# fernandezdaniel/MOBOCMF

Hardware: AMD Instinct MI355X
Metric: ELBO steps/sec (MFDGP d=8 M=512 N=8192 S=8) (higher is better)
Workload: dtype f64

## Files before the change

### mobocmf_amd/csrc/api.hip

```cpp
#include "common.h"

static const mobocmf_tuning kDefaultTuning = {(uint32_t)sizeof(mobocmf_tuning), 384, 512, 0, 0, 1024, 32, 0, 1, 0};
static thread_local const mobocmf_tuning* t_tuning = nullptr;
static thread_local void* const* t_probe = nullptr;
const mobocmf_tuning& tune() { return t_tuning ? *t_tuning : kDefaultTuning; }
bool tuning_ok(const mobocmf_tuning* t) {
    if (!t) return true;
    return t->struct_size == sizeof(mobocmf_tuning) && t->small_gemm_max >= 1 && t->small_gemm_max <= 512 &&
           t->small_panel_max >= 1 && t->small_panel_max <= 512 && (t->tile_rows == 0 || t->tile_rows == 64 || t->tile_rows == 128) &&
           t->pair_mode >= 0 && t->pair_mode <= 2 && t->mid_gemm_max >= 0 && t->mid_gemm_max <= 4096 &&
           (t->mid_gemm_waves == 4 || t->mid_gemm_waves == 8 || t->mid_gemm_waves == 32) &&
           (t->syrk_workgroups == 0 || (t->syrk_workgroups >= 16 && t->syrk_workgroups <= 4096)) &&
           (t->sparse_backward == 0 || t->sparse_backward == 1) && (t->potrf_cols == 0 || t->potrf_cols == 1 || t->potrf_cols == 4);
}
TuneScope::TuneScope(const mobocmf_tuning* t, void* const* probe) : prev_t(t_tuning), prev_p(t_probe) {
    t_tuning = t;
    t_probe = probe;
}
TuneScope::~TuneScope() {
    t_tuning = prev_t;
    t_probe = prev_p;
}
void probe_at(int i, hipStream_t s) {
    if (t_probe && i < MOBOCMF_PROBE_EVENTS && t_probe[i]) (void)hipEventRecord((hipEvent_t)t_probe[i], s);
// ... 344 lines not shown
    TRY(launch_moments_bwd_prep(g_mean, g_var, P.knn, P.q, P.varraw, desc->branch, desc->min_var, D.N, Np, B.gmu, B.gv,
                                B.gv2, B.cgv, nclamped, c.nclamped ? 1 : 0, (int32_t*)act, s));
    int da_parts = 0;
    {
        GemmArgs ga = gemm_args(c.U, Mp, P.C, Np, B.dA, Np, Mp, Np, Mp, TRI_LOWER_A, 2.0);
        ga.bscale = B.gv; ga.epi = EPI_DA; ga.avec = c.a; ga.gmu = B.gmu; ga.cgv = B.cgv; ga.Aaux = P.A;
        ga.Kreal = D.M;
        ga.rowdot_part = desc->params_const ? nullptr : B.dapart;
        ga.colact = act;
        ga.rm = panel_tile_rows(Mp, Np);
        set_pairing(ga);
        probe_at(3, s);
        TRY(launch_gemm(ga, false, 1, s));
        probe_at(4, s);
        da_parts = desc->params_const ? 0 : gemm_rowdot_parts(ga);
    }
    if (!desc->params_const) {
        probe_at(5, s);
        if (desc->branch == 0) TRY(weighted_syrk_pair(P.A, Np, B.gv, B.cgv, Mp, Np, B.slabs, B.slabs2, c.H, Hc, nclamped, act, s));
        else TRY(weighted_syrk(P.A, Np, B.gv, Mp, Np, B.slabs, c.H, nullptr, nullptr, act, s));
        probe_at(6, s);
    }
    {
        GemmArgs ga = gemm_args(c.LinvT, Mp, B.dA, Np, B.dK, Np, Mp, Np, Mp, TRI_UPPER_A, 1.0);
        ga.Kreal = D.M;
        ga.rm = panel_tile_rows(Mp, Np);
        set_pairing(ga);
        ga.colact = act;
        probe_at(7, s);
        TRY(launch_gemm(ga, false, 1, s));
        probe_at(8, s);
    }
    GramArgs g = {};
    g.kind = desc->kind; g.d = desc->d; g.zdiv = 1; g.Zx = Zx; g.zf = zf; g.M = D.M; g.hyp = hyp; g.Mp = Mp;
    g.xdiv = desc->xdiv; g.x = x; g.f = f; g.nbase = D.nbase;
    g.ldk = Np; g.Np = Np; g.G = B.dK; g.gknn = B.cgv; g.colact = act;
    g.hyp_part = B.hyp_part; g.df_part = B.df_part; g.dzf_part = B.dzf_part; g.dx_part = B.dx_part;
    TRY(launch_gram_bwd(g, desc->want_dx != 0, s));
    probe_at(10, s);
    SumTask tk[5];
    int nt = 0;
    if (da_parts > 0) tk[nt++] = {B.dapart, da_parts, Mp, nullptr, 0, 0, c.da, Mp, 0};
    tk[nt++] = {B.hyp_part, (int64_t)D.ggrid_mn.x * D.ggrid_mn.y, D.H, nullptr, 0, 0, g_hyp, D.H, 0};
    if (desc->kind == 1) {
        tk[nt++] = {B.df_part, D.ggrid_mn.y, Np, nullptr, 0, 0, g_f, D.N, 0};
        tk[nt++] = {B.dzf_part, D.ggrid_mn.x, Mp, nullptr, 0, 0, g_zf, D.M, 0};
    }
    if (desc->want_dx)
        tk[nt++] = {B.dx_part, D.ggrid_mn.y, D.nbase * desc->d, nullptr, 0, 0, g_x, D.nbase * desc->d, 0};
    return launch_sum_partials_multi(tk, nt, s);
}

int chain_backward(int n, const ChainWs& c, int64_t zs, const ChainIO& io, const Dims& D, const bool* zero, const int* acc,
                   const bool* fold, hipStream_t s) {
    const int Mp = D.Mp;
    const int64_t mm = (int64_t)Mp * Mp;
    double *G1 = c.W[0], *F = c.W[1], *Gm = c.W[2], *dU = c.W[3], *Wn = c.W[4], *T1 = c.W[5], *T4 = c.W[6], *T2 = c.W[7];
    bool any_clamp_branch = false;
    for (int z = 0; z < n; ++z) {
        if (zero[z]) {
            TRY(launch_zero32(c.H + z * zs, mm * 2, s));
            TRY(launch_zero32(c.Hc + z * zs, mm * 2, s));
            TRY(launch_zero32(c.da + z * zs, (int64_t)Mp * 2, s));
        }
        any_clamp_branch = any_clamp_branch || io.desc[z]->branch == 0;
    }
    for (int z = 0; z < n; ++z)
        if (io.desc[z]->branch != 0 && !zero[z] && (n > 1 || any_clamp_branch))
            TRY(launch_copy_block(c.H + z * zs, Mp, c.Hc + z * zs, Mp, Mp, Mp, s));
    const double* Hc = (n == 1 && io.desc[0]->branch != 0) ? c.H : c.Hc;
    {
        GemmArgs g1 = gemm_args(c.UT, Mp, c.H, Mp, G1, Mp, Mp, Mp, Mp, TRI_UPPER_A, 1.0);
        g1.Kreal = D.M;
        TRY(chain_gemm(g1, false, c, n, zs, s));
        TRY(launch_chain_glue_z(G1, Hc, c.U, c.da, c.a, io.g_kl, D.M, Mp, F, dU, c.da_tot, Wn, n, zs, s));
        GemmArgs gw = gemm_args(F, Mp, c.UT, Mp, Wn, Mp, Mp, Mp, Mp, TRI_UPPER_B, -1.0);
        gw.accumulate = 1;
        gw.Kreal = D.M;
        TRY(chain_gemm(gw, false, c, n, zs, s));
    }
    {
        GemmArgs ga = gemm_args(c.LinvT, Mp, dU, Mp, T1, Mp, Mp, Mp, Mp, TRI_UPPER_A | TRI_LOWER_B, 1.0);
        ga.lower_out = 1;
        ga.Kreal = D.M;
        GemmArgs gb = gemm_args(c.LinvT, Mp, Wn, Mp, T4, Mp, Mp, Mp, Mp, TRI_UPPER_A, 1.0);
        gb.Kreal = D.M;
        if (n > 1) {
            ga.zlayers = gb.zlayers = n;
            ga.zsA = ga.zsB = ga.zsC = gb.zsA = gb.zsB = gb.zsC = zs;
        }
        TRY(launch_gemm_auto_pair(ga, gb, c.slabs, c.slab_elems, s));
        TRY(launch_chain_outputs_z(T1, c.LSp, c.LinvT, c.da_tot, D.M, Mp, io.g_kl, io.g_LS, io.g_m, n, zs, s));
    }
    {
        GemmArgs gc = gemm_args(T4, Mp, c.Linv, Mp, T2, Mp, Mp, Mp, Mp, TRI_LOWER_B, 1.0);
        gc.Kreal = D.M;
        TRY(chain_gemm(gc, false, c, n, zs, s));
        TRY(launch_symmetrize_z(T2, Mp, Gm, n, zs, s));
    }
    SumTask tk[2 * MAX_ZL];
    int nt = 0;
    for (int z = 0; z < n; ++z) {
        const mobocmf_layer_desc* d = io.desc[z];
        GramArgs g = kmm_gram(d, D, io.Zx[z], io.zf[z], io.hyp[z]);
        g.G = Gm + z * zs; g.gknn = nullptr;
        g.hyp_part = c.hyp_part2 + z * zs; g.df_part = c.df_part2 + z * zs; g.dzf_part = c.dzf_part2 + z * zs;
        g.dx_part = nullptr;
        TRY(launch_gram_bwd(g, false, s));
        const int H = hyp_len(d->kind, d->d);
        tk[nt++] = {g.hyp_part, (int64_t)D.ggrid_mm.x * D.ggrid_mm.y, H, nullptr, 0, 0, io.g_hyp[z], H, acc[z]};
        if (d->kind == 1) {
            if (fold[z])
                tk[nt++] = {g.df_part, D.ggrid_mm.y, Mp, g.dzf_part, D.ggrid_mm.x, Mp, io.g_m[z - 1], D.M, 1,
                            acc[z] ? io.g_zf[z] : nullptr};
            else
                tk[nt++] = {g.df_part, D.ggrid_mm.y, Mp, g.dzf_part, D.ggrid_mm.x, Mp, io.g_zf[z], D.M, acc[z], nullptr};
        }
    }
    return launch_sum_partials_multi(tk, nt, s);
}

bool gram_rows_shape_ok(int32_t kind, int32_t d, int64_t n1, int64_t nbase2, int32_t xdiv) {
    return (kind == 0 || kind == 1) && d >= 1 && d <= MOBOCMF_MAX_D && n1 >= 1 && nbase2 >= 1 && xdiv >= 1 &&
           xdiv <= MOBOCMF_MAX_XDIV && n1 <= (int64_t)65535 * 64 && nbase2 <= 0x7fffffff;
}
int64_t gram_rows_part_elems(int32_t d, int64_t n1, int64_t nbase2, int32_t xdiv, int64_t* chunks_out = nullptr) {
    int64_t chunks;
    int groups, wb;
    gram_rows_geometry(n1, nbase2, xdiv, &chunks, &groups, &wb);
    if (chunks_out) *chunks_out = chunks;
    return chunks * n1 * d;
}
int gram_rows_partials(int kind, int d, const double* x1, const double* f1, int64_t n1, const double* x2, const double* f2,
                       int64_t nbase2, int xdiv, const double* hyp, const double* G, int64_t ldk, const int32_t* colact,
                       int symmetric, double* part, hipStream_t s) {
    GramRowsArgs g = {};
    g.kind = kind; g.d = d; g.xdiv = xdiv; g.symmetric = symmetric;
    g.x1 = x1; g.f1 = f1; g.n1 = n1; g.x2 = x2; g.f2 = f2; g.nbase2 = nbase2;
    g.hyp = hyp; g.G = G; g.ldk = ldk; g.colact = colact; g.part = part;
    return launch_gram_bwd_rows(g, s);
}
bool ranges_overlap(const void* a, size_t na, const void* b, size_t nb) {
    const uintptr_t pa = (uintptr_t)a, pb = (uintptr_t)b;
    return a && b && pa < pb + nb && pb < pa + na;
}
int panel_rows_partials(const mobocmf_layer_desc* desc, const Dims& D, const PanelBwd& B, const double* x, const double* f,
                        const double* Zx, const double* zf, const double* hyp, double* part, hipStream_t s) {
    return gram_rows_partials(desc->kind, desc->d, Zx, zf, D.M, x, f, D.nbase, desc->xdiv, hyp, B.dK, D.Np,
                              tune().sparse_backward ? B.blkact : nullptr, 0, part, s);
}
int chain_rows_partials(const mobocmf_layer_desc* desc, const Dims& D, const ChainWs& c, int z, int64_t zs, const double* Zx,
                        const double* zf, const double* hyp, double* part, hipStream_t s) {
    return gram_rows_partials(desc->kind, desc->d, Zx, zf, D.M, Zx, zf, D.M, 1, hyp, c.W[2] + z * zs, D.Mp, nullptr, 1, part, s);
}

bool same_chain_shape(int n, const mobocmf_layer_desc* const* d) {
    for (int z = 0; z < n; ++z)
        if (!valid_desc(d[z]) || d[z]->M != d[0]->M) return false;
    return true;
}

}

namespace {
int64_t gcd64(int64_t a, int64_t b) { while (b) { int64_t t = a % b; a = b; b = t; } return a; }
int64_t covpanel_cols(const mobocmf_layer_desc* d, int64_t Np) {
    const int64_t l = (int64_t)TILE / gcd64(TILE, d->xdiv) * d->xdiv;
    int64_t w = l * (2048 / l > 1 ? 2048 / l : 1);
    return w < Np ? w : Np;
}
struct CovWs { double *Knm, *AT, *CT, *Cv; };
// ... 45 lines not shown
    if (!valid_desc(desc) || desc->params_const || !x || !Zx || !hyp || !m || !L_S || !mean || !var || !kl || !info || !saved ||
        !scratch)
        return MOBOCMF_BAD_ARG;
    TuneScope tune_scope(desc->tuning, desc->probe_events);
    if (desc->kind == 1 && (!zf || !f)) return MOBOCMF_BAD_ARG;
    hipStream_t s = (hipStream_t)stream;
    Dims D = dims_of(desc);
    ChainWs c = {};
    PanelSaved P;
    PanelFwd F;
    if (!carve_single_saved(saved, saved_bytes, D, c, P) || !carve_single_fwd(scratch, scratch_bytes, D, c, F))
        return MOBOCMF_WORKSPACE_TOO_SMALL;
    ChainIO io = {};
    io.desc = &desc; io.Zx = &Zx; io.zf = &zf; io.hyp = &hyp; io.m = &m; io.L_S = &L_S; io.kl = &kl; io.info = &info;
    TRY(chain_forward(1, c, 0, io, D, s));
    return panel_forward(desc, D, c, P, F, x, f, Zx, zf, hyp, mean, var, s);
}

static int layer_backward_impl(const mobocmf_layer_desc* desc, const double* x, const double* f, const double* Zx,
                               const double* zf, const double* hyp, const double* m, const double* L_S,
                               const double* g_mean, const double* g_var, const double* g_kl, double* g_f, double* g_zf,
                               double* g_hyp, double* g_m, double* g_LS, double* g_x, void* saved, size_t saved_bytes,
                               void* scratch, size_t scratch_bytes, bool want_z, double* g_Zx, void* zws, size_t zws_bytes,
                               mobocmf_stream_t stream) {
    if ((want_z && (!g_Zx || !zws)) || !valid_desc(desc) || desc->params_const || !x || !Zx || !hyp || !g_mean || !g_var || !g_kl || !g_hyp || !g_m || !g_LS ||
        (desc->want_dx && !g_x) || !saved || !scratch)
        return MOBOCMF_BAD_ARG;
    TuneScope tune_scope(desc->tuning, desc->probe_events);
    if (desc->kind == 1 && (!zf || !g_zf || !f || !g_f)) return MOBOCMF_BAD_ARG;
    hipStream_t s = (hipStream_t)stream;
    Dims D = dims_of(desc);
    ChainWs c = {};
    PanelSaved P;
    PanelBwd B;
    if (!carve_single_saved(saved, saved_bytes, D, c, P) || !carve_single_bwd(scratch, scratch_bytes, D, desc, c, B))
        return MOBOCMF_WORKSPACE_TOO_SMALL;
    Bump bz(zws, zws_bytes);
    int64_t chp = 0, chc = 0;
    double *zp = nullptr, *zc = nullptr;
    if (want_z) {
        if (ranges_overlap(zws, zws_bytes, scratch, scratch_bytes) || ranges_overlap(zws, zws_bytes, saved, saved_bytes))
            return MOBOCMF_BAD_ARG;
        zp = bz.take(gram_rows_part_elems(desc->d, D.M, D.nbase, desc->xdiv, &chp));
        zc = bz.take(gram_rows_part_elems(desc->d, D.M, D.M, 1, &chc));
        if (!bz.ok) return MOBOCMF_WORKSPACE_TOO_SMALL;
    }
    TRY(panel_backward(desc, D, c, P, B, x, f, Zx, zf, hyp, g_mean, g_var, g_f, g_zf, g_hyp, g_x, s));
    if (want_z) TRY(panel_rows_partials(desc, D, B, x, f, Zx, zf, hyp, zp, s));
    ChainIO io = {};
    io.desc = &desc; io.Zx = &Zx; io.zf = &zf; io.hyp = &hyp; io.m = &m; io.L_S = &L_S;
    io.g_kl = &g_kl; io.g_zf = &g_zf; io.g_hyp = &g_hyp; io.g_m = &g_m; io.g_LS = &g_LS;
    const bool zero = false, fold = false;
    const int acc = 1;
    TRY(chain_backward(1, c, 0, io, D, &zero, &acc, &fold, s));
    if (!want_z) return MOBOCMF_OK;
    TRY(chain_rows_partials(desc, D, c, 0, 0, Zx, zf, hyp, zc, s));
    const int64_t len = (int64_t)D.M * desc->d;
    const SumTask tk = {zp, chp, len, zc, chc, len, g_Zx, len, 0, nullptr};
    return launch_sum_partials_multi(&tk, 1, s);
}

int mobocmf_layer_backward(const mobocmf_layer_desc* desc, const double* x, const double* f, const double* Zx,
                           const double* zf, const double* hyp, const double* m, const double* L_S,
                           const double* g_mean, const double* g_var, const double* g_kl, double* g_f, double* g_zf,
                           double* g_hyp, double* g_m, double* g_LS, double* g_x, void* saved, size_t saved_bytes,
                           void* scratch, size_t scratch_bytes, mobocmf_stream_t stream) {
    return layer_backward_impl(desc, x, f, Zx, zf, hyp, m, L_S, g_mean, g_var, g_kl, g_f, g_zf, g_hyp, g_m, g_LS, g_x, saved,
                               saved_bytes, scratch, scratch_bytes, false, nullptr, nullptr, 0, stream);
}

int mobocmf_layer_backward_z(const mobocmf_layer_desc* desc, const double* x, const double* f, const double* Zx,
                             const double* zf, const double* hyp, const double* m, const double* L_S,
                             const double* g_mean, const double* g_var, const double* g_kl, double* g_f, double* g_zf,
                             double* g_hyp, double* g_m, double* g_LS, double* g_x, double* g_Zx, void* saved,
                             size_t saved_bytes, void* scratch, size_t scratch_bytes, void* zws, size_t zws_bytes,
                             mobocmf_stream_t stream) {
    return layer_backward_impl(desc, x, f, Zx, zf, hyp, m, L_S, g_mean, g_var, g_kl, g_f, g_zf, g_hyp, g_m, g_LS, g_x, saved,
                               saved_bytes, scratch, scratch_bytes, true, g_Zx, zws, zws_bytes, stream);
}

int mobocmf_inducing_grad_workspace_bytes(const mobocmf_layer_desc* desc, size_t* panel_bytes, size_t* chain_bytes) {
    if (!valid_desc(desc) || !panel_bytes || !chain_bytes) return MOBOCMF_BAD_ARG;
    Dims D = dims_of(desc);
    Bump bp(nullptr, ~(size_t)0 >> 1), bc(nullptr, ~(size_t)0 >> 1);
    bp.take(gram_rows_part_elems(desc->d, D.M, D.nbase, desc->xdiv));
    bc.take(gram_rows_part_elems(desc->d, D.M, D.M, 1));
    *panel_bytes = bp.off;
    *chain_bytes = bc.off;
    return MOBOCMF_OK;
}

int mobocmf_chain_block_bytes(const mobocmf_layer_desc* desc, size_t* block_bytes, size_t* state_bytes) {
    if (!valid_desc(desc) || !block_bytes) return MOBOCMF_BAD_ARG;
    TuneScope tune_scope(desc->tuning, desc->probe_events);
    Dims D = dims_of(desc);
    ChainWs c;
    size_t st = 0, used = 0;
    carve_chain_block(nullptr, ~(size_t)0 >> 1, D, c, &st, &used);
    *block_bytes = used;
    if (state_bytes) *state_bytes = st;
    return MOBOCMF_OK;
}

int mobocmf_panel_workspace_bytes(const mobocmf_layer_desc* desc, size_t* saved_bytes, size_t* scratch_bytes) {
    if (!valid_desc(desc) || !saved_bytes || !scratch_bytes) return MOBOCMF_BAD_ARG;
    TuneScope tune_scope(desc->tuning, desc->probe_events);
    Dims D = dims_of(desc);
// ... 21 lines not shown
    if (blocks_bytes / (size_t)n < block_stride) return MOBOCMF_WORKSPACE_TOO_SMALL;
    for (int z = 0; z < n; ++z)
        if (!Zx[z] || !hyp[z] || !m[z] || !L_S[z] || !kl[z] || !info[z] || (desc[z]->kind == 1 && !zf[z])) return MOBOCMF_BAD_ARG;
    Dims D = dims_of(desc[0]);
    ChainWs c = {};
    if (!carve_chain_block(blocks, block_stride, D, c)) return MOBOCMF_WORKSPACE_TOO_SMALL;
    ChainIO io = {};
    io.desc = desc; io.Zx = Zx; io.zf = zf; io.hyp = hyp; io.m = m; io.L_S = L_S; io.kl = kl; io.info = info;
    return chain_forward(n, c, (int64_t)(block_stride / sizeof(double)), io, D, (hipStream_t)stream);
}

static int layers_chain_backward_impl(int32_t n, const mobocmf_layer_desc* const* desc, const double* const* Zx,
                                      const double* const* zf, const double* const* hyp, const double* const* g_kl,
                                      const int32_t* had_panel, double* const* g_zf, double* const* g_hyp, double* const* g_m,
                                      double* const* g_LS, void* blocks, size_t block_stride, size_t blocks_bytes, bool want_z,
                                      double* const* g_Zx, void* zws, size_t zws_bytes, mobocmf_stream_t stream) {
    if ((want_z && (!g_Zx || !zws)) || n < 1 || n > MAX_ZL || !desc || !Zx || !zf || !hyp || !g_kl || !had_panel || !g_zf || !g_hyp || !g_m || !g_LS ||
        !blocks || (block_stride & 255))
        return MOBOCMF_BAD_ARG;
    if (!same_chain_shape(n, desc)) return MOBOCMF_BAD_ARG;
    TuneScope tune_scope(desc[0]->tuning);
    if (blocks_bytes / (size_t)n < block_stride) return MOBOCMF_WORKSPACE_TOO_SMALL;
    bool zero[MAX_ZL], fold[MAX_ZL];
    int acc[MAX_ZL];
    for (int z = 0; z < n; ++z) {
        if (!Zx[z] || !hyp[z] || !g_kl[z] || !g_hyp[z] || !g_m[z] || !g_LS[z] || (desc[z]->kind == 1 && (!zf[z] || !g_zf[z])))
            return MOBOCMF_BAD_ARG;
        const int hp = had_panel[z] & 3;
        if (hp == 3 || (had_panel[z] & ~7)) return MOBOCMF_BAD_ARG;
        zero[z] = hp == 0;
        acc[z] = hp == 2 ? 1 : 0;
        fold[z] = (had_panel[z] & 4) != 0;
        if (fold[z] && (z == 0 || desc[z]->kind != 1)) return MOBOCMF_BAD_ARG;
    }
    Dims D = dims_of(desc[0]);
    ChainWs c = {};
    if (!carve_chain_block(blocks, block_stride, D, c)) return MOBOCMF_WORKSPACE_TOO_SMALL;
    ChainIO io = {};
    io.desc = desc; io.Zx = Zx; io.zf = zf; io.hyp = hyp;
    io.g_kl = g_kl; io.g_zf = g_zf; io.g_hyp = g_hyp; io.g_m = g_m; io.g_LS = g_LS;
    const int64_t zs = (int64_t)(block_stride / sizeof(double));
    hipStream_t s = (hipStream_t)stream;
    Bump bz(zws, zws_bytes);
    double* zc[MAX_ZL] = {};
    int64_t chc[MAX_ZL] = {};
    if (want_z) {
        if (ranges_overlap(zws, zws_bytes, blocks, blocks_bytes)) return MOBOCMF_BAD_ARG;
        for (int z = 0; z < n; ++z) {
            if (!g_Zx[z]) return MOBOCMF_BAD_ARG;
            zc[z] = bz.take(gram_rows_part_elems(desc[z]->d, D.M, D.M, 1, &chc[z]));
        }
        if (!bz.ok) return MOBOCMF_WORKSPACE_TOO_SMALL;
    }
    TRY(chain_backward(n, c, zs, io, D, zero, acc, fold, s));
    if (!want_z) return MOBOCMF_OK;
    SumTask tk[MAX_ZL];
    for (int z = 0; z < n; ++z) {
        TRY(chain_rows_partials(desc[z], D, c, z, zs, Zx[z], zf[z], hyp[z], zc[z], s));
        const int64_t len = (int64_t)D.M * desc[z]->d;
        tk[z] = {zc[z], chc[z], len, nullptr, 0, 0, g_Zx[z], len, 0, nullptr};
    }
    return launch_sum_partials_multi(tk, n, s);
}

int mobocmf_layers_chain_backward(int32_t n, const mobocmf_layer_desc* const* desc, const double* const* Zx,
                                  const double* const* zf, const double* const* hyp, const double* const* g_kl,
                                  const int32_t* had_panel, double* const* g_zf, double* const* g_hyp, double* const* g_m,
                                  double* const* g_LS, void* blocks, size_t block_stride, size_t blocks_bytes,
                                  mobocmf_stream_t stream) {
    return layers_chain_backward_impl(n, desc, Zx, zf, hyp, g_kl, had_panel, g_zf, g_hyp, g_m, g_LS, blocks, block_stride,
                                      blocks_bytes, false, nullptr, nullptr, 0, stream);
}

int mobocmf_layers_chain_backward_z(int32_t n, const mobocmf_layer_desc* const* desc, const double* const* Zx,
                                    const double* const* zf, const double* const* hyp, const double* const* g_kl,
                                    const int32_t* had_panel, double* const* g_zf, double* const* g_hyp, double* const* g_m,
                                    double* const* g_LS, double* const* g_Zx, void* blocks, size_t block_stride,
                                    size_t blocks_bytes, void* zws, size_t zws_bytes, mobocmf_stream_t stream) {
    return layers_chain_backward_impl(n, desc, Zx, zf, hyp, g_kl, had_panel, g_zf, g_hyp, g_m, g_LS, blocks, block_stride,
                                      blocks_bytes, true, g_Zx, zws, zws_bytes, stream);
}

int mobocmf_layer_panel_forward(const mobocmf_layer_desc* desc, const double* x, const double* f, const double* Zx,
                                const double* zf, const double* hyp, double* mean, double* var, void* chain_block,
                                size_t block_bytes, void* saved, size_t saved_bytes, void* scratch, size_t scratch_bytes,
                                mobocmf_stream_t stream) {
    if (!valid_desc(desc) || !x || !Zx || !hyp || !mean || !var || !chain_block || !saved || !scratch) return MOBOCMF_BAD_ARG;
    TuneScope tune_scope(desc->tuning, desc->probe_events);
    if (desc->kind == 1 && (!zf || !f)) return MOBOCMF_BAD_ARG;
    Dims D = dims_of(desc);
    ChainWs c = {};
    if (!carve_panel_chain(desc, chain_block, block_bytes, D, c)) return MOBOCMF_WORKSPACE_TOO_SMALL;
    Bump bs(saved, saved_bytes), bf(scratch, scratch_bytes);
    PanelSaved P;
    PanelFwd F;
    carve_panel_saved(bs, D, P);
    carve_panel_fwd(bf, D, F);
    if (!bs.ok || !bf.ok) return MOBOCMF_WORKSPACE_TOO_SMALL;
    return panel_forward(desc, D, c, P, F, x, f, Zx, zf, hyp, mean, var, (hipStream_t)stream);
}

static int layer_panel_backward_impl(const mobocmf_layer_desc* desc, const double* x, const double* f, const double* Zx,
                                     const double* zf, const double* hyp, const double* g_mean, const double* g_var,
                                     double* g_f, double* g_zf, double* g_hyp, double* g_x, void* chain_block,
                                     size_t block_bytes, void* saved, size_t saved_bytes, void* scratch, size_t scratch_bytes,
                                     bool want_z, double* g_Zx, void* zws, size_t zws_bytes, mobocmf_stream_t stream) {
    if ((want_z && (!g_Zx || !zws || (desc && desc->params_const))) || !valid_desc(desc) || !x || !Zx || !hyp || !g_mean || !g_var || !g_hyp || !chain_block || !saved || !scratch ||
// ... 542 lines not shown
```

### mobocmf_amd/csrc/common.h

```cpp
#pragma once
#include <hip/hip_runtime.h>
#include <stdint.h>

#include "../../include/mobocmf_hip.h"

#define TILE 128
#define NB 64

static inline int64_t round_up(int64_t v, int64_t m) { return (v + m - 1) / m * m; }

#define HIP_TRY(expr)                                   \
    do {                                                \
        hipError_t _e = (expr);                         \
        if (_e != hipSuccess) return MOBOCMF_HIP_ERROR; \
    } while (0)

const mobocmf_tuning& tune();
bool tuning_ok(const mobocmf_tuning* t);
void probe_at(int i, hipStream_t s);
struct TuneScope {
    const mobocmf_tuning* prev_t;
    void* const* prev_p;
    explicit TuneScope(const mobocmf_tuning* t, void* const* probe = nullptr);
    ~TuneScope();
// ... 33 lines not shown
    const int32_t* skip_if_zero;
    const int32_t* dual_flag;
    const double* bscale2;
    double* C2;
    const int32_t* colact;
    const int32_t* kact;
    int epi;
    double* colsq_part;
    double* coldot_part;
    const double* avec;
    const double* gmu;
    const double* cgv;
    const double* Aaux;
};

int launch_gemm(const GemmArgs& g, bool B_T, int splitk, hipStream_t s);
int gemm_nt_slabs(const GemmArgs& g, int splitk);
bool gemm_nt_is_small(const GemmArgs& g);
int gemm_rowdot_parts(const GemmArgs& g);
int gemm_colstat_rows(const GemmArgs& g);
int launch_gemm_auto(const GemmArgs& g, bool B_T, double* ws, int64_t ws_elems, hipStream_t s);
int launch_gemm_auto_pair(const GemmArgs& a, const GemmArgs& b, double* ws, int64_t ws_elems, hipStream_t s);

#define MAX_ZL 4

struct GramArgs {
    int kind, d, xdiv, zdiv;
    const double* x;
    const double* f;
    int64_t nbase;
    const double* Zx;
    const double* zf;
    int M;
    const double* hyp;
    double* K;
    int64_t ldk;
    int Mp;
    int64_t Np;
    double* knn;
    double jitter;
    int is_kmm;
    int gm;
    const double* G;
    const double* gknn;
    double* hyp_part;
    double* df_part;
    double* dzf_part;
    double* dx_part;
    const int32_t* colact;
};
int launch_gram_fwd(const GramArgs& g, hipStream_t s);
int launch_gram_bwd(const GramArgs& g, bool want_dx, hipStream_t s);
void gram_grid(const GramArgs& g, dim3* grid);
struct SumTask {
    const double* part; int64_t P, stride;
    const double* part2; int64_t P2, stride2;
    double* out; int64_t len; int accumulate;
    const double* extra;
};
int launch_sum_partials_multi(const SumTask* tasks, int n, hipStream_t s);

struct GramRowsArgs {
    int kind, d, xdiv;
    int symmetric;
    const double* x1;
    const double* f1;
    int64_t n1;
    const double* x2;
    const double* f2;
    int64_t nbase2;
    const double* hyp;
    const double* G;
    int64_t ldk;
    const int32_t* colact;
    double* part;
    int wb;
};
void gram_rows_geometry(int64_t n1, int64_t nbase2, int xdiv, int64_t* chunks, int* groups, int* wb);
int launch_gram_bwd_rows(const GramRowsArgs& g, hipStream_t s);

int launch_trtri(const double* L, int64_t ld, int Mp, const double* Dinv, double* Linv, double* T, double* ws,
                 int64_t ws_elems, hipStream_t s);
int launch_potrf_z(double* A, int64_t ld, int Mp, int M, double* Dinv, double* Ld, int32_t* const* info, int nz, int64_t zs,
                   double* zero0, double* zero1, void* sync, int* inverse_done, hipStream_t s);
int launch_trtri_z(const double* L, int64_t ld, int Mp, const double* Dinv, double* Linv, double* T, double* ws,
                   int64_t ws_elems, int nz, int64_t zs, hipStream_t s);

int launch_zero32(void* ptr, int64_t nwords, hipStream_t s);
int launch_pad_vec(const double* src, int64_t n, double* dst, int64_t np, hipStream_t s);
int launch_gemv_rows(const double* Mat, int64_t ld, const double* vec, double* out, int rows, int64_t cols, double scale,
                     int accumulate, hipStream_t s);
int launch_moments_finish(const double* qpart, const double* mupart, const double* rpart, int nrb, int64_t Np, int64_t N,
                          const double* knn, int branch, double min_var, double* q, double* r, double* varraw,
                          double* mean, double* var, int32_t* zero_word, hipStream_t s);
int launch_moments_bwd_prep(const double* g_mean, const double* g_var, const double* knn, const double* q,
                            const double* varraw, int branch, double min_var, int64_t N, int64_t Np, double* gmu,
                            double* gv, double* gv2, double* cgv, int32_t* nclamped, int zeroed, int32_t* blkact, hipStream_t s);
int launch_reduce_slabs_sym(const double* slabs, int64_t slab_stride, int nslab, int nslab_diag, double* out, int Mp, const int32_t* flag,
                            const double* fallback, hipStream_t s);
int launch_reduce_slabs_sym2(const double* slabs, const double* slabs2, int64_t slab_stride, int nslab, int nslab_diag,
                             double* out, double* out2, int Mp, const int32_t* flag, hipStream_t s);
int launch_copy_block(const double* src, int64_t lds, double* dst, int64_t ldd, int64_t rows, int64_t cols, hipStream_t s);
int launch_mf_combine(const double* Ks, const double* Kn, int64_t ld, const double* s1, const double* s2, const int32_t* l1,
                      const int32_t* l2, const double* ntab, int64_t n1, int64_t n2, double diag, double* out, int64_t ldo,
                      int64_t rows_p, int64_t cols_p, hipStream_t s);
int launch_copy_pad_identity(const double* src, int64_t lds, int n, double* dst, int np, hipStream_t s);
// ... 60 lines not shown
```

### mobocmf_amd/csrc/elementwise.hip

```cpp
#include "common.h"

#define LOG_2PI 1.8378770664093454835606594728112

__device__ __forceinline__ double wave_sum(double v) {
    v += __shfl_xor(v, 1);
    v += __shfl_xor(v, 2);
    v += __shfl_xor(v, 4);
    v += __shfl_xor(v, 8);
    v += __shfl_xor(v, 16);
    v += __shfl_xor(v, 32);
    return v;
}

__device__ __forceinline__ double block_sum(double v, double* sh) {
    v = wave_sum(v);
    const int lane = threadIdx.x & 63, wave = threadIdx.x >> 6;
    __syncthreads();
    if (lane == 0) sh[wave] = v;
    __syncthreads();
    double t = 0.0;
    if (threadIdx.x == 0)
        for (int w = 0; w < (int)(blockDim.x >> 6); ++w) t += sh[w];
    return t;
}
// ... 785 lines not shown
    int64_t t = (int64_t)blockIdx.x * blockDim.x + threadIdx.x;
    if (t >= T) return;
    double sm = 0.0, s2 = 0.0;
    for (int s = 0; s < S; ++s) {
        double m = mu_t[t * S + s];
        sm += m;
        s2 += var_t[t * S + s] + m * m;
    }
    sm /= S;
    s2 /= S;
    mus[t] = sm;
    vars[t] = s2 - sm * sm;
}
__global__ void acq_bwd_kernel(const double* mu_t, const double* gmus, const double* gvars, double* gmu_t,
                               double* gvar_t, int64_t T, int S) {
    int64_t t = (int64_t)blockIdx.x * blockDim.x + threadIdx.x;
    if (t >= T) return;
    double sm = 0.0;
    for (int s = 0; s < S; ++s) sm += mu_t[t * S + s];
    sm /= S;
    const double gm = gmus ? gmus[t] : 0.0, gvv = gvars ? gvars[t] : 0.0;
    for (int s = 0; s < S; ++s) {
        double m = mu_t[t * S + s];
        gmu_t[t * S + s] = gm / S + gvv * (2.0 * m / S - 2.0 * sm / S);
        gvar_t[t * S + s] = gvv / S;
    }
}
__global__ void jes_kernel(const double* vu, const double* vc, double* acq, int64_t T) {
    int64_t t = (int64_t)blockIdx.x * blockDim.x + threadIdx.x;
    if (t >= T) return;
    double v = log(vu[t]) - log(vc[t]);
    acq[t] = 0.5 * (v > 0.0 ? v : 0.0);
}
__global__ void adam_kernel(double* p, const double* g, double* m, double* v, const double* mask, int64_t n, double lr,
                            double b1, double b2, double eps, double bc1, double bc2_sqrt) {
    int64_t i = (int64_t)blockIdx.x * blockDim.x + threadIdx.x;
    if (i >= n) return;
    if (mask && mask[i] == 0.0) return;
    double gi = g[i];
    double mi = b1 * m[i] + (1.0 - b1) * gi;
    double vi = b2 * v[i] + (1.0 - b2) * gi * gi;
    m[i] = mi;
    v[i] = vi;
    p[i] -= (lr / bc1) * mi / (sqrt(vi) / bc2_sqrt + eps);
}

#define ADAM_MAX_TENSORS 40
struct AdamTable {
    double* p[ADAM_MAX_TENSORS];
    const double* g[ADAM_MAX_TENSORS];
    double* m[ADAM_MAX_TENSORS];
    double* v[ADAM_MAX_TENSORS];
    int64_t n[ADAM_MAX_TENSORS];
};
__global__ void adam_multi_kernel(AdamTable t, double lr, double b1, double b2, double eps, const int64_t* steps_done) {
    const int64_t step = steps_done[0] + 1;
    const int ti = blockIdx.y;
    const int64_t n = t.n[ti];
    const double bc1 = 1.0 - pow(b1, (double)step), bc2s = sqrt(1.0 - pow(b2, (double)step));
    double* p = t.p[ti];
    const double* g = t.g[ti];
    double* m = t.m[ti];
    double* v = t.v[ti];
    for (int64_t i = (int64_t)blockIdx.x * blockDim.x + threadIdx.x; i < n; i += (int64_t)gridDim.x * blockDim.x) {
        const double gi = g[i];
        const double mi = b1 * m[i] + (1.0 - b1) * gi;
        const double vi = b2 * v[i] + (1.0 - b2) * gi * gi;
        m[i] = mi;
        v[i] = vi;
        p[i] -= (lr / bc1) * mi / (sqrt(vi) / bc2s + eps);
    }
}
__global__ void adam_count_kernel(int64_t* steps_done) { steps_done[0] += 1; }

__global__ void shortcut_var_fwd_kernel(const double* L, int M, double min_var, double* var) {
    const int row = blockIdx.x * 4 + (threadIdx.x >> 6), lane = threadIdx.x & 63;
    if (row >= M) return;
    double s = 0.0;
    for (int j = lane; j <= row; j += 64) {
        const double v = L[(int64_t)row * M + j];
        s += v * v;
    }
    s = wave_sum(s);
    if (lane == 0) var[row] = s > min_var ? s : min_var;
}
__global__ void shortcut_var_bwd_kernel(const double* L, const double* var, const double* g, int M, double min_var,
                                        double* gL) {
    int64_t idx = (int64_t)blockIdx.x * blockDim.x + threadIdx.x;
    if (idx >= (int64_t)M * M) return;
    const int i = (int)(idx / M), j = (int)(idx % M);
    gL[idx] = (j <= i && var[i] > min_var) ? 2.0 * L[idx] * g[i] : 0.0;
}

#define COMBINE_MAX 8
struct CombineTable { const double* a[COMBINE_MAX]; const double* b[COMBINE_MAX]; };
__global__ void elbo_combine_fwd_kernel(CombineTable t, int na, int nb, double scale, double* out) {
    double sa = 0.0, sb = 0.0;
    for (int i = 0; i < na; ++i) sa += t.a[i][0];
    for (int j = 0; j < nb; ++j) sb += t.b[j][0];
    out[0] = sa - scale * sb;
    out[1] = scale * sb;
}
__global__ void elbo_combine_bwd_kernel(const double* g_elbo, const double* g_skl, double scale, double* g) {
    const double ge = g_elbo ? g_elbo[0] : 0.0, gs = g_skl ? g_skl[0] : 0.0;
    g[0] = ge;
    g[1] = scale * (gs - ge);
}

extern "C" {

int mobocmf_shortcut_var_forward(const double* L_S, int32_t M, double min_var, double* var, mobocmf_stream_t stream) {
    if (!L_S || !var || M < 1) return MOBOCMF_BAD_ARG;
    hipLaunchKernelGGL(shortcut_var_fwd_kernel, dim3((unsigned)((M + 3) / 4)), dim3(256), 0, (hipStream_t)stream, L_S, M,
                       min_var, var);
    return CHECK_LAUNCH();
}

int mobocmf_shortcut_var_backward(const double* L_S, const double* var, const double* g_var, int32_t M, double min_var,
                                  double* g_LS, mobocmf_stream_t stream) {
    if (!L_S || !var || !g_var || !g_LS || M < 1) return MOBOCMF_BAD_ARG;
    hipLaunchKernelGGL(shortcut_var_bwd_kernel, GRID1((int64_t)M * M), 0, (hipStream_t)stream, L_S, var, g_var, M, min_var,
                       g_LS);
    return CHECK_LAUNCH();
}

int mobocmf_elbo_combine_forward(int32_t n_data, const double* const* data_terms, int32_t n_kl, const double* const* kls,
                                 double scale, double* out2, mobocmf_stream_t stream) {
    if (n_data < 0 || n_kl < 0 || n_data > COMBINE_MAX || n_kl > COMBINE_MAX || !out2 || (n_data && !data_terms) ||
        (n_kl && !kls))
        return MOBOCMF_BAD_ARG;
    CombineTable t = {};
    for (int i = 0; i < n_data; ++i) { if (!data_terms[i]) return MOBOCMF_BAD_ARG; t.a[i] = data_terms[i]; }
    for (int j = 0; j < n_kl; ++j) { if (!kls[j]) return MOBOCMF_BAD_ARG; t.b[j] = kls[j]; }
    hipLaunchKernelGGL(elbo_combine_fwd_kernel, dim3(1), dim3(1), 0, (hipStream_t)stream, t, n_data, n_kl, scale, out2);
    return CHECK_LAUNCH();
}

int mobocmf_elbo_combine_backward(const double* g_elbo, const double* g_skl, double scale, double* g2,
                                  mobocmf_stream_t stream) {
    if (!g2) return MOBOCMF_BAD_ARG;
    hipLaunchKernelGGL(elbo_combine_bwd_kernel, dim3(1), dim3(1), 0, (hipStream_t)stream, g_elbo, g_skl, scale, g2);
    return CHECK_LAUNCH();
}

int mobocmf_adam_multi(int32_t n_tensors, double* const* params, const double* const* grads, double* const* exp_avg,
                       double* const* exp_avg_sq, const int64_t* sizes, double lr, double beta1, double beta2, double eps,
                       int64_t* step_state, mobocmf_stream_t stream) {
    if (n_tensors < 0 || !step_state || (n_tensors && (!params || !grads || !exp_avg || !exp_avg_sq || !sizes)))
        return MOBOCMF_BAD_ARG;
    hipStream_t s = (hipStream_t)stream;
    for (int base = 0; base < n_tensors; base += ADAM_MAX_TENSORS) {
        AdamTable t;
        int cnt = n_tensors - base < ADAM_MAX_TENSORS ? n_tensors - base : ADAM_MAX_TENSORS;
        int64_t nmax = 0;
        for (int i = 0; i < cnt; ++i) {
            t.p[i] = params[base + i]; t.g[i] = grads[base + i]; t.m[i] = exp_avg[base + i]; t.v[i] = exp_avg_sq[base + i];
            t.n[i] = sizes[base + i];
            if (t.n[i] < 0 || !t.p[i] || !t.g[i] || !t.m[i] || !t.v[i]) return MOBOCMF_BAD_ARG;
            if (t.n[i] > nmax) nmax = t.n[i];
        }
        int64_t bx = (nmax + 1023) / 1024;
        if (bx < 1) bx = 1;
        if (bx > 4096) bx = 4096;
        hipLaunchKernelGGL(adam_multi_kernel, dim3((unsigned)bx, (unsigned)cnt), dim3(256), 0, s, t, lr, beta1, beta2, eps,
                           (const int64_t*)step_state);
    }
    hipLaunchKernelGGL(adam_count_kernel, dim3(1), dim3(1), 0, s, step_state);
    return CHECK_LAUNCH();
}

#define PACK_MAX_TENSORS 16
struct PackTable {
    const double* raw[PACK_MAX_TENSORS];
    double* g_raw[PACK_MAX_TENSORS];
    const double* g_src[PACK_MAX_TENSORS];
    int32_t off[PACK_MAX_TENSORS + 1];
};
__global__ void softplus_pack_kernel(PackTable t, int nt, double* out) {
    for (int e = threadIdx.x; e < t.off[nt]; e += blockDim.x) {
        int ti = 0;
        while (e >= t.off[ti + 1]) ++ti;
        const double x = t.raw[ti][e - t.off[ti]];
        out[e] = x > 20.0 ? x : log1p(exp(x));
    }
}
__global__ void softplus_pack_bwd_kernel(PackTable t, int nt, const double* g_out) {
    for (int e = threadIdx.x; e < t.off[nt]; e += blockDim.x) {
        int ti = 0;
        while (e >= t.off[ti + 1]) ++ti;
        const double x = t.raw[ti][e - t.off[ti]];
        t.g_raw[ti][e - t.off[ti]] = x > 20.0 ? g_out[e] : g_out[e] / (1.0 + exp(-x));
    }
}
__global__ void softplus_pack_bwd_v_kernel(PackTable t, int nt) {
    for (int e = threadIdx.x; e < t.off[nt]; e += blockDim.x) {
        int ti = 0;
        while (e >= t.off[ti + 1]) ++ti;
        const int k = e - t.off[ti];
        const double x = t.raw[ti][k];
        const double g = t.g_src[ti] ? t.g_src[ti][k] : 0.0;
        t.g_raw[ti][k] = x > 20.0 ? g : g / (1.0 + exp(-x));
    }
}
static int fill_pack_table(PackTable& t, int32_t n, const double* const* raw, double* const* g_raw, const int32_t* sizes) {
    if (n < 1 || n > PACK_MAX_TENSORS || !raw || !sizes) return MOBOCMF_BAD_ARG;
    t.off[0] = 0;
    for (int i = 0; i < n; ++i) {
        if (!raw[i] || sizes[i] < 1 || (g_raw && !g_raw[i])) return MOBOCMF_BAD_ARG;
        t.raw[i] = raw[i];
        t.g_raw[i] = g_raw ? g_raw[i] : nullptr;
        t.off[i + 1] = t.off[i] + sizes[i];
    }
    return MOBOCMF_OK;
}
int mobocmf_softplus_pack(int32_t n_tensors, const double* const* raw, const int32_t* sizes, double* out,
                          mobocmf_stream_t stream) {
    PackTable t;
    if (!out) return MOBOCMF_BAD_ARG;
// ... 374 lines not shown
```

### mobocmf_amd/csrc/gram.hip

```cpp
#include "common.h"

#define GT 128
#define GM 32


typedef double v2f64_t __attribute__((ext_vector_type(2)));

template <int KIND, int DB, int XD>
__global__ __launch_bounds__(GT) void gram_fwd_kernel(GramArgs g) {
    __shared__ __attribute__((aligned(16))) double stg[XD ? (GT / 64) * 64 * (XD + 2) : 1];
    __shared__ double zs[GM][DB];
    __shared__ double zfs[GM];
    __shared__ double il1[DB], il2[DB];
    const int d = g.d;
    const int tid = threadIdx.x;
    const int gm = g.gm;
    const int m0 = blockIdx.y * gm;
    const double* hyp = g.hyp;
    double a1, af = 0, nu = 0, a2 = 0, ilf = 0;
    if (KIND == 0) {
        a1 = hyp[0];
        if (tid < DB) il1[tid] = tid < d ? 1.0 / hyp[1 + tid] : 0.0;
    } else {
        a1 = hyp[0]; af = hyp[1]; nu = hyp[2]; a2 = hyp[3]; ilf = 1.0 / hyp[4];
// ... 412 lines not shown
    int64_t nb_cols = (g.Np + g.xdiv - 1) / g.xdiv;
    int64_t gx = (nb_cols + GT - 1) / GT;
    int gm = GM;
    while (gm > GM / 4 && gx * (g.Mp / gm) < 1024) gm /= 2;
    if (fwd && g.is_kmm)
        while (gm > 2 && gx * (g.Mp / gm) < 4096) gm /= 2;
    return gm;
}
void gram_grid(const GramArgs& g, dim3* grid) {
    int64_t nb_cols = (g.Np + g.xdiv - 1) / g.xdiv;
    *grid = dim3((unsigned)((nb_cols + GT - 1) / GT), (unsigned)(g.Mp / gram_rows_per_block(g)), 1);
}

int launch_gram_fwd(const GramArgs& g0, hipStream_t s) {
    GramArgs g = g0;
    g.gm = gram_rows_per_block(g0, true);
    if (g.d < 1 || g.d > 32) return MOBOCMF_BAD_ARG;
    dim3 grid;
    gram_grid(g, &grid);
    grid.y = (unsigned)(g.Mp / g.gm);
    const int db = d_bucket(g.d);
#define GF(K, D, X) hipLaunchKernelGGL((gram_fwd_kernel<K, D, X>), grid, dim3(GT), 0, s, g)
    const bool vec_ok = g.kind == 1 && !g.is_kmm && ((uintptr_t)g.f % 16 == 0) && ((uintptr_t)g.K % 16 == 0) && (g.ldk % 2 == 0);
    if (g.kind == 0) { if (db == 2) GF(0, 2, 0); else if (db == 8) GF(0, 8, 0); else GF(0, 32, 0); }
    else if (vec_ok && g.xdiv == 8) { if (db == 2) GF(1, 2, 8); else if (db == 8) GF(1, 8, 8); else GF(1, 32, 8); }
    else if (vec_ok && g.xdiv == 16) { if (db == 2) GF(1, 2, 16); else if (db == 8) GF(1, 8, 16); else GF(1, 32, 16); }
    else { if (db == 2) GF(1, 2, 0); else if (db == 8) GF(1, 8, 0); else GF(1, 32, 0); }
#undef GF
    return hipGetLastError() == hipSuccess ? MOBOCMF_OK : MOBOCMF_HIP_ERROR;
}

int launch_gram_bwd(const GramArgs& g0, bool want_dx, hipStream_t s) {
    GramArgs g = g0;
    g.gm = gram_rows_per_block(g0);
    if (g.d < 1 || g.d > 32) return MOBOCMF_BAD_ARG;
    dim3 grid;
    gram_grid(g, &grid);
    const int db = d_bucket(g.d);
    if (g.xdiv > 48) return MOBOCMF_BAD_ARG;
    const size_t shm = g.kind == 1 ? (size_t)g.xdiv * GT * sizeof(double) : 0;
#define GB(K, D, X)                                                                                    \
    do {                                                                                               \
        if (want_dx) hipLaunchKernelGGL((gram_bwd_kernel<K, D, true, X>), grid, dim3(GT), (X) ? 0 : shm, s, g);   \
        else hipLaunchKernelGGL((gram_bwd_kernel<K, D, false, X>), grid, dim3(GT), (X) ? 0 : shm, s, g);          \
    } while (0)
    const bool vec_ok = g.kind == 1 && ((uintptr_t)g.f % 16 == 0) && ((uintptr_t)g.G % 16 == 0) && (g.ldk % 2 == 0);
    if (g.kind == 0) { if (db == 2) GB(0, 2, 0); else if (db == 8) GB(0, 8, 0); else GB(0, 32, 0); }
    else if (vec_ok && g.xdiv == 8) { if (db == 2) GB(1, 2, 8); else if (db == 8) GB(1, 8, 8); else GB(1, 32, 8); }
    else if (vec_ok && g.xdiv == 16) { if (db == 2) GB(1, 2, 16); else if (db == 8) GB(1, 8, 16); else GB(1, 32, 16); }
    else { if (db == 2) GB(1, 2, 0); else if (db == 8) GB(1, 8, 0); else GB(1, 32, 0); }
#undef GB
    return hipGetLastError() == hipSuccess ? MOBOCMF_OK : MOBOCMF_HIP_ERROR;
}
```

Before: 1102.

## Fuse Kmm gram backward across layers with symmetric tiles reading T2 directly

```diff
diff --git a/mobocmf_amd/csrc/api.hip b/mobocmf_amd/csrc/api.hip
--- a/mobocmf_amd/csrc/api.hip
+++ b/mobocmf_amd/csrc/api.hip
@@ -420,7 +420,7 @@
 }
 
 int chain_backward(int n, const ChainWs& c, int64_t zs, const ChainIO& io, const Dims& D, const bool* zero, const int* acc,
-                   const bool* fold, hipStream_t s) {
+                   const bool* fold, bool want_gm, hipStream_t s) {
     const int Mp = D.Mp;
     const int64_t mm = (int64_t)Mp * Mp;
     double *G1 = c.W[0], *F = c.W[1], *Gm = c.W[2], *dU = c.W[3], *Wn = c.W[4], *T1 = c.W[5], *T4 = c.W[6], *T2 = c.W[7];
@@ -464,27 +464,28 @@
         GemmArgs gc = gemm_args(T4, Mp, c.Linv, Mp, T2, Mp, Mp, Mp, Mp, TRI_LOWER_B, 1.0);
         gc.Kreal = D.M;
         TRY(chain_gemm(gc, false, c, n, zs, s));
-        TRY(launch_symmetrize_z(T2, Mp, Gm, n, zs, s));
-    }
+        if (want_gm) TRY(launch_symmetrize_z(T2, Mp, Gm, n, zs, s));
+    }
+    const int wgs = gram_kmm_workgroups(D.M, (int64_t)D.ggrid_mm.x * D.ggrid_mm.y), ntr = gram_kmm_tile_rows(D.M);
+    GramKmmArgs ka = {};
+    ka.n = n; ka.M = D.M; ka.Mp = Mp;
     SumTask tk[2 * MAX_ZL];
     int nt = 0;
     for (int z = 0; z < n; ++z) {
         const mobocmf_layer_desc* d = io.desc[z];
-        GramArgs g = kmm_gram(d, D, io.Zx[z], io.zf[z], io.hyp[z]);
-        g.G = Gm + z * zs; g.gknn = nullptr;
-        g.hyp_part = c.hyp_part2 + z * zs; g.df_part = c.df_part2 + z * zs; g.dzf_part = c.dzf_part2 + z * zs;
-        g.dx_part = nullptr;
-        TRY(launch_gram_bwd(g, false, s));
+        GramKmmLayer& l = ka.l[z];
+        l.kind = d->kind; l.d = d->d; l.Zx = io.Zx[z]; l.zf = io.zf[z]; l.hyp = io.hyp[z]; l.T2 = T2 + z * zs;
+        l.hyp_part = c.hyp_part2 + z * zs; l.zf_part = c.df_part2 + z * zs;
         const int H = hyp_len(d->kind, d->d);
-        tk[nt++] = {g.hyp_part, (int64_t)D.ggrid_mm.x * D.ggrid_mm.y, H, nullptr, 0, 0, io.g_hyp[z], H, acc[z]};
+        tk[nt++] = {l.hyp_part, wgs, H, nullptr, 0, 0, io.g_hyp[z], H, acc[z]};
         if (d->kind == 1) {
             if (fold[z])
-                tk[nt++] = {g.df_part, D.ggrid_mm.y, Mp, g.dzf_part, D.ggrid_mm.x, Mp, io.g_m[z - 1], D.M, 1,
-                            acc[z] ? io.g_zf[z] : nullptr};
+                tk[nt++] = {l.zf_part, ntr, Mp, nullptr, 0, 0, io.g_m[z - 1], D.M, 1, acc[z] ? io.g_zf[z] : nullptr};
             else
-                tk[nt++] = {g.df_part, D.ggrid_mm.y, Mp, g.dzf_part, D.ggrid_mm.x, Mp, io.g_zf[z], D.M, acc[z], nullptr};
+                tk[nt++] = {l.zf_part, ntr, Mp, nullptr, 0, 0, io.g_zf[z], D.M, acc[z], nullptr};
         }
     }
+    TRY(launch_gram_bwd_kmm(ka, wgs, s));
     return launch_sum_partials_multi(tk, nt, s);
 }
 
@@ -636,7 +637,7 @@
     io.g_kl = &g_kl; io.g_zf = &g_zf; io.g_hyp = &g_hyp; io.g_m = &g_m; io.g_LS = &g_LS;
     const bool zero = false, fold = false;
     const int acc = 1;
-    TRY(chain_backward(1, c, 0, io, D, &zero, &acc, &fold, s));
+    TRY(chain_backward(1, c, 0, io, D, &zero, &acc, &fold, want_z, s));
     if (!want_z) return MOBOCMF_OK;
     TRY(chain_rows_partials(desc, D, c, 0, 0, Zx, zf, hyp, zc, s));
     const int64_t len = (int64_t)D.M * desc->d;
@@ -764,7 +765,7 @@
         }
         if (!bz.ok) return MOBOCMF_WORKSPACE_TOO_SMALL;
     }
-    TRY(chain_backward(n, c, zs, io, D, zero, acc, fold, s));
+    TRY(chain_backward(n, c, zs, io, D, zero, acc, fold, want_z, s));
     if (!want_z) return MOBOCMF_OK;
     SumTask tk[MAX_ZL];
     for (int z = 0; z < n; ++z) {
diff --git a/mobocmf_amd/csrc/common.h b/mobocmf_amd/csrc/common.h
--- a/mobocmf_amd/csrc/common.h
+++ b/mobocmf_amd/csrc/common.h
@@ -109,6 +109,19 @@
 int launch_gram_fwd(const GramArgs& g, hipStream_t s);
 int launch_gram_bwd(const GramArgs& g, bool want_dx, hipStream_t s);
 void gram_grid(const GramArgs& g, dim3* grid);
+struct GramKmmLayer {
+    int kind, d;
+    const double* Zx;
+    const double* zf;
+    const double* hyp;
+    const double* T2;
+    double* hyp_part;
+    double* zf_part;
+};
+struct GramKmmArgs { GramKmmLayer l[MAX_ZL]; int n, M, Mp; };
+int gram_kmm_tile_rows(int M);
+int gram_kmm_workgroups(int M, int64_t max_wgs);
+int launch_gram_bwd_kmm(const GramKmmArgs& a, int wgs, hipStream_t s);
 struct SumTask {
     const double* part; int64_t P, stride;
     const double* part2; int64_t P2, stride2;
diff --git a/mobocmf_amd/csrc/elementwise.hip b/mobocmf_amd/csrc/elementwise.hip
--- a/mobocmf_amd/csrc/elementwise.hip
+++ b/mobocmf_amd/csrc/elementwise.hip
@@ -861,17 +861,27 @@
     double* m[ADAM_MAX_TENSORS];
     double* v[ADAM_MAX_TENSORS];
     int64_t n[ADAM_MAX_TENSORS];
+    int blk0[ADAM_MAX_TENSORS + 1];
+    int cnt;
 };
 __global__ void adam_multi_kernel(AdamTable t, double lr, double b1, double b2, double eps, const int64_t* steps_done) {
-    const int64_t step = steps_done[0] + 1;
-    const int ti = blockIdx.y;
+    __shared__ double bc[2];
+    if (threadIdx.x < 64) {
+        const int64_t step = steps_done[0] + 1;
+        const double c1 = 1.0 - pow(b1, (double)step), c2 = sqrt(1.0 - pow(b2, (double)step));
+        if (threadIdx.x == 0) { bc[0] = c1; bc[1] = c2; }
+    }
+    int ti = 0;
+    while (ti + 1 < t.cnt && (int)blockIdx.x >= t.blk0[ti + 1]) ++ti;
     const int64_t n = t.n[ti];
-    const double bc1 = 1.0 - pow(b1, (double)step), bc2s = sqrt(1.0 - pow(b2, (double)step));
+    const int nb = t.blk0[ti + 1] - t.blk0[ti];
     double* p = t.p[ti];
     const double* g = t.g[ti];
     double* m = t.m[ti];
     double* v = t.v[ti];
-    for (int64_t i = (int64_t)blockIdx.x * blockDim.x + threadIdx.x; i < n; i += (int64_t)gridDim.x * blockDim.x) {
+    __syncthreads();
+    const double bc1 = bc[0], bc2s = bc[1];
+    for (int64_t i = (int64_t)((int)blockIdx.x - t.blk0[ti]) * blockDim.x + threadIdx.x; i < n; i += (int64_t)nb * blockDim.x) {
         const double gi = g[i];
         const double mi = b1 * m[i] + (1.0 - b1) * gi;
         const double vi = b2 * v[i] + (1.0 - b2) * gi * gi;
@@ -961,18 +971,21 @@
     for (int base = 0; base < n_tensors; base += ADAM_MAX_TENSORS) {
         AdamTable t;
         int cnt = n_tensors - base < ADAM_MAX_TENSORS ? n_tensors - base : ADAM_MAX_TENSORS;
-        int64_t nmax = 0;
+        int nb = 0;
         for (int i = 0; i < cnt; ++i) {
             t.p[i] = params[base + i]; t.g[i] = grads[base + i]; t.m[i] = exp_avg[base + i]; t.v[i] = exp_avg_sq[base + i];
             t.n[i] = sizes[base + i];
             if (t.n[i] < 0 || !t.p[i] || !t.g[i] || !t.m[i] || !t.v[i]) return MOBOCMF_BAD_ARG;
-            if (t.n[i] > nmax) nmax = t.n[i];
-        }
-        int64_t bx = (nmax + 1023) / 1024;
-        if (bx < 1) bx = 1;
-        if (bx > 4096) bx = 4096;
-        hipLaunchKernelGGL(adam_multi_kernel, dim3((unsigned)bx, (unsigned)cnt), dim3(256), 0, s, t, lr, beta1, beta2, eps,
-                           (const int64_t*)step_state);
+            int64_t bx = (t.n[i] + 1023) / 1024;
+            if (bx > 4096) bx = 4096;
+            t.blk0[i] = nb;
+            nb += (int)bx;
+        }
+        for (int i = cnt; i <= ADAM_MAX_TENSORS; ++i) t.blk0[i] = nb;
+        t.cnt = cnt;
+        if (nb > 0)
+            hipLaunchKernelGGL(adam_multi_kernel, dim3((unsigned)nb), dim3(256), 0, s, t, lr, beta1, beta2, eps,
+                               (const int64_t*)step_state);
     }
     hipLaunchKernelGGL(adam_count_kernel, dim3(1), dim3(1), 0, s, step_state);
     return CHECK_LAUNCH();
diff --git a/mobocmf_amd/csrc/gram.hip b/mobocmf_amd/csrc/gram.hip
--- a/mobocmf_amd/csrc/gram.hip
+++ b/mobocmf_amd/csrc/gram.hip
@@ -488,3 +488,201 @@
 #undef GB
     return hipGetLastError() == hipSuccess ? MOBOCMF_OK : MOBOCMF_HIP_ERROR;
 }
+
+#define KT 32
+#define KTHR 256
+static_assert(KT * KT / KTHR == 4, "the tile body selects among four prefetched elements");
+
+template <int DB>
+struct KmmShared {
+    double zr[KT][DB + 1];
+    double zc[DB > 8 ? KT : 1][DB + 1];
+    double tt[KT][KT + 1];
+    double zfr[KT], il1[DB], il2[DB];
+    double rowacc[KT], colp[KTHR / KT][KT];
+    double red[KTHR / 64][8 + 2 * DB];
+};
+
+template <int KIND, int DB>
+__device__ __forceinline__ void gram_bwd_kmm_tiles(const GramKmmLayer& L, const int M, const int Mp, KmmShared<DB>& sm) {
+    const int d = L.d;
+    const int tid = threadIdx.x, lane = tid & 63, wave = tid >> 6;
+    const int j = tid & (KT - 1), q = tid / KT;
+    const int nt = (M + KT - 1) / KT, tiles = nt * (nt + 1) / 2;
+    const double* hyp = L.hyp;
+    double a1, af = 0, nu = 0, a2 = 0, ilf = 0;
+    if (KIND == 0) {
+        a1 = hyp[0];
+        if (tid < DB) sm.il1[tid] = tid < d ? 1.0 / hyp[1 + tid] : 0.0;
+    } else {
+        a1 = hyp[0]; af = hyp[1]; nu = hyp[2]; a2 = hyp[3]; ilf = 1.0 / hyp[4];
+        if (tid < DB) { sm.il1[tid] = tid < d ? 1.0 / hyp[5 + tid] : 0.0; sm.il2[tid] = tid < d ? 1.0 / hyp[5 + d + tid] : 0.0; }
+    }
+    double aL1[DB], aL2[KIND == 1 ? DB : 1];
+#pragma unroll
+    for (int k = 0; k < DB; ++k) {
+        aL1[k] = 0.0;
+        if (KIND == 1) aL2[k] = 0.0;
+    }
+    double s_a1 = 0, s_af = 0, s_nu = 0, s_a2 = 0, s_lsf = 0;
+
+    for (int t = blockIdx.x; t < tiles; t += gridDim.x) {
+        int I = (int)((sqrtf(8.0f * (float)t + 1.0f) - 1.0f) * 0.5f);
+        while ((I + 1) * (I + 2) / 2 <= t) ++I;
+        while (I * (I + 1) / 2 > t) --I;
+        const int J = t - I * (I + 1) / 2;
+        const int m0 = I * KT, n0 = J * KT;
+        __syncthreads();
+        for (int e = tid; e < KT * DB; e += KTHR) {
+            const int mm = e / DB, k = e % DB;
+            sm.zr[mm][k] = (m0 + mm < M && k < d) ? L.Zx[(int64_t)(m0 + mm) * d + k] : 0.0;
+        }
+        if (KIND == 1 && tid < KT) sm.zfr[tid] = (m0 + tid < M) ? L.zf[m0 + tid] : 0.0;
+#pragma unroll
+        for (int r = 0; r < KT * KT / KTHR; ++r) {
+            const int jj = q + (KTHR / KT) * r;
+            sm.tt[jj][j] = (n0 + jj < M && m0 + j < M) ? L.T2[(int64_t)(n0 + jj) * Mp + m0 + j] : 0.0;
+        }
+        const int n = n0 + j;
+        const bool creal = n < M;
+        double xr[DB > 8 ? 1 : DB];
+        if (DB > 8) {
+            for (int e = tid; e < KT * DB; e += KTHR) {
+                const int nn = e / DB, k = e % DB;
+                sm.zc[nn][k] = (n0 + nn < M && k < d) ? L.Zx[(int64_t)(n0 + nn) * d + k] : 0.0;
+            }
+        } else {
+#pragma unroll
+            for (int k = 0; k < (DB > 8 ? 1 : DB); ++k) xr[k] = (creal && k < d) ? L.Zx[(int64_t)n * d + k] : 0.0;
+        }
+        const double fn = (KIND == 1 && creal) ? L.zf[n] : 0.0;
+        double gd[KT * KT / KTHR];
+#pragma unroll
+        for (int r = 0; r < KT * KT / KTHR; ++r) {
+            const int m = m0 + q + (KTHR / KT) * r;
+            gd[r] = (creal && m < M && m >= n) ? L.T2[(int64_t)m * Mp + n] : 0.0;
+        }
+        __syncthreads();
+
+        double colv = 0.0;
+#pragma unroll 1
+        for (int r = 0; r < KT * KT / KTHR; ++r) {
+            const int i = q + (KTHR / KT) * r;
+            const int m = m0 + i;
+            double Gw = r == 0 ? gd[0] : r == 1 ? gd[1] : r == 2 ? gd[2] : gd[3];
+            if (creal && m < M && m > n) Gw += sm.tt[j][i];
+            double d1 = 0.0, d2 = 0.0;
+#pragma unroll
+            for (int k = 0; k < DB; ++k) {
+                const double df = (DB > 8 ? sm.zc[DB > 8 ? j : 0][k] : xr[DB > 8 ? 0 : k]) - sm.zr[i][k];
+                const double t1 = df * sm.il1[k];
+                d1 += t1 * t1;
+                if (KIND == 1) { const double t2 = df * sm.il2[k]; d2 += t2 * t2; }
+            }
+            const double E1 = exp(-0.5 * d1);
+            double W1, W2 = 0.0, rowv = 0.0;
+            if (KIND == 0) {
+                s_a1 += Gw * E1;
+                W1 = Gw * a1 * E1;
+            } else {
+                const double E2 = exp(-0.5 * d2);
+                const double zfm = sm.zfr[i];
+                const double fd = (fn - zfm) * ilf;
+                const double Ef = exp(-0.5 * fd * fd);
+                const double GaE1 = Gw * a1 * E1;
+                const double inner = nu * zfm * fn + af * Ef;
+                const double Tb = GaE1 * af * ilf * Ef * fd;
+                s_a1 += Gw * E1 * inner;
+                s_nu += GaE1 * zfm * fn;
+                s_af += GaE1 * Ef;
+                s_lsf += Tb * fd;
+                s_a2 += Gw * E2;
+                W1 = GaE1 * inner;
+                W2 = Gw * a2 * E2;
+                rowv = GaE1 * nu * fn + Tb;
+                colv += GaE1 * nu * zfm - Tb;
+            }
+#pragma unroll
+            for (int k = 0; k < DB; ++k) {
+                const double df = (DB > 8 ? sm.zc[DB > 8 ? j : 0][k] : xr[DB > 8 ? 0 : k]) - sm.zr[i][k];
+                const double t1 = df * sm.il1[k];
+                aL1[k] += W1 * t1 * t1;
+                if (KIND == 1) { const double t2 = df * sm.il2[k]; aL2[k] += W2 * t2 * t2; }
+            }
+            if (KIND == 1) {
+                rowv += __shfl_xor(rowv, 1);
+                rowv += __shfl_xor(rowv, 2);
+                rowv += __shfl_xor(rowv, 4);
+                rowv += __shfl_xor(rowv, 8);
+                rowv += __shfl_xor(rowv, 16);
+                if (j == 0) sm.rowacc[i] = rowv;
+            }
+        }
+        if (KIND == 1) {
+            sm.colp[q][j] = colv;
+            __syncthreads();
+            if (tid < KT) {
+                double cv = 0.0;
+#pragma unroll
+                for (int p = 0; p < KTHR / KT; ++p) cv += sm.colp[p][tid];
+                if (I == J) L.zf_part[(int64_t)I * Mp + m0 + tid] = sm.rowacc[tid] + cv;
+                else {
+                    L.zf_part[(int64_t)J * Mp + m0 + tid] = sm.rowacc[tid];
+                    L.zf_part[(int64_t)I * Mp + n0 + tid] = cv;
+                }
+            }
+        }
+    }
+    const int H = (KIND == 0) ? 1 + d : 5 + 2 * d;
+    {
+        double v;
+        v = wave_sum(s_a1); if (lane == 0) sm.red[wave][0] = v;
+        if (KIND == 1) {
+            v = wave_sum(s_af); if (lane == 0) sm.red[wave][1] = v;
+            v = wave_sum(s_nu); if (lane == 0) sm.red[wave][2] = v;
+            v = wave_sum(s_a2); if (lane == 0) sm.red[wave][3] = v;
+            v = wave_sum(s_lsf); if (lane == 0) sm.red[wave][4] = v;
+        }
+#pragma unroll
+        for (int k = 0; k < DB; ++k) {
+            if (k < d) {
+                v = wave_sum(aL1[k]);
+                if (lane == 0) sm.red[wave][(KIND == 0 ? 1 : 5) + k] = v * sm.il1[k];
+                if (KIND == 1) {
+                    v = wave_sum(aL2[k]);
+                    if (lane == 0) sm.red[wave][5 + d + k] = v * sm.il2[k];
+                }
+            }
+        }
+    }
+    __syncthreads();
+    if (tid < H) L.hyp_part[(int64_t)blockIdx.x * H + tid] = (sm.red[0][tid] + sm.red[1][tid]) + (sm.red[2][tid] + sm.red[3][tid]);
+}
+
+template <int DB>
+__global__ __launch_bounds__(KTHR) void gram_bwd_kmm_kernel(GramKmmArgs a) {
+    __shared__ KmmShared<DB> sm;
+    const GramKmmLayer& L = a.l[blockIdx.y];
+    if (L.kind == 0) gram_bwd_kmm_tiles<0, DB>(L, a.M, a.Mp, sm);
+    else gram_bwd_kmm_tiles<1, DB>(L, a.M, a.Mp, sm);
+}
+
+int gram_kmm_tile_rows(int M) { return (M + KT - 1) / KT; }
+int gram_kmm_workgroups(int M, int64_t max_wgs) {
+    const int64_t nt = gram_kmm_tile_rows(M), tiles = nt * (nt + 1) / 2;
+    return (int)(tiles < max_wgs ? tiles : max_wgs);
+}
+
+int launch_gram_bwd_kmm(const GramKmmArgs& a, int wgs, hipStream_t s) {
+    if (a.n < 1 || a.n > MAX_ZL || wgs < 1 || a.M < 1 || a.Mp < a.M) return MOBOCMF_BAD_ARG;
+    int db = 2;
+    for (int z = 0; z < a.n; ++z) {
+        if (a.l[z].d < 1 || a.l[z].d > 32) return MOBOCMF_BAD_ARG;
+        if (d_bucket(a.l[z].d) > db) db = d_bucket(a.l[z].d);
+    }
+    const dim3 grid((unsigned)wgs, (unsigned)a.n);
+    if (db == 2) hipLaunchKernelGGL((gram_bwd_kmm_kernel<2>), grid, dim3(KTHR), 0, s, a);
+    else if (db == 8) hipLaunchKernelGGL((gram_bwd_kmm_kernel<8>), grid, dim3(KTHR), 0, s, a);
+    else hipLaunchKernelGGL((gram_bwd_kmm_kernel<32>), grid, dim3(KTHR), 0, s, a);
+    return hipGetLastError() == hipSuccess ? MOBOCMF_OK : MOBOCMF_HIP_ERROR;
+}
```

After: 1110 (median of 6 runs). Within noise of the previous version (+0.8%).
